# fugue-project/fugue

Hardware: NVIDIA H100
Metric: transform() rows/sec, hash-partitioned (num=256) identity map, 8-col table (higher is better)
Workload: dtype int64+f64 (byte moves; u64 hash arithmetic)

## Files before the change

fugue_b200/csrc/fb_partition.cu:

```cuda
#include <stdlib.h>

#include <mutex>

#include "fb_common.cuh"

namespace {

constexpr int kBlock = 512;
constexpr int kItems = 8;
constexpr int kTile = kBlock * kItems;
constexpr int kWarps = kBlock / 32;
constexpr int kCtasPerSm = 2;

struct FbCols {
  const void* src[FB_MAX_COLS];
  void* dst[FB_MAX_COLS];
  int32_t width[FB_MAX_COLS];
  int32_t ncols;
};

struct ChunkGeom {
  int64_t nrows;
  int64_t full_rows;
  int64_t tiles_per_chunk;
// ... 433 lines not shown

template <bool kSingleU64, int kBits, bool kAll8>
__global__ void __launch_bounds__(kBlock, kCtasPerSm)
fb_scatter_kernel(FbKeys keys, FbDiv dv, uint32_t num, ChunkGeom g, int chunk0,
                  const uint32_t* __restrict__ chunk_base, const int64_t* __restrict__ part_offsets,
                  FbCols cols) {
  extern __shared__ __align__(128) uint64_t smem64[];
  TileCtx cx;
  cx.nbp = nb_padded(num);
  cx.buf = smem64;
  cx.delta = (uint32_t*)(smem64 + 2 * kTile);
  cx.cursor = cx.delta + cx.nbp;
  cx.bin_start = cx.cursor + cx.nbp;
  cx.cnt = cx.bin_start + cx.nbp;
  cx.scanw = cx.cnt + kWarps * cx.nbp;
  cx.pid_sorted = (uint16_t*)(cx.scanw + 32);

  const int chunk = chunk0 + (int)blockIdx.x;
  int64_t chunk_row0, chunk_row1;
  chunk_range(g, chunk, chunk_row0, chunk_row1);

  for (uint32_t b = threadIdx.x; b < cx.nbp; b += kBlock)
    cx.cursor[b] = b < num ? (uint32_t)part_offsets[b] + chunk_base[(size_t)chunk * num + b] : 0u;
  for (uint32_t i = threadIdx.x; i < (uint32_t)kWarps * cx.nbp; i += kBlock) cx.cnt[i] = 0;
  __syncthreads();

  int phase = 0;
  for (int64_t tile_row0 = chunk_row0; tile_row0 < chunk_row1; tile_row0 += kTile) {
    const int64_t left = chunk_row1 - tile_row0;
    if (left >= kTile)
      scatter_tile<kSingleU64, kBits, true, kAll8>(keys, dv, num, cols, cx, tile_row0, kTile, phase);
    else
      scatter_tile<kSingleU64, kBits, false, kAll8>(keys, dv, num, cols, cx, tile_row0, (int)left, phase);
  }
}

constexpr int kSwcMaxCols = 8;
constexpr uint32_t kSwcMaxNum = 256;

__device__ __forceinline__ uint32_t smem_u32(const void* p) { return (uint32_t)__cvta_generic_to_shared(p); }

__device__ __forceinline__ void mbar_init(uint32_t bar, uint32_t count) {
  asm volatile("mbarrier.init.shared::cta.b64 [%0], %1;" ::"r"(bar), "r"(count) : "memory");
}
__device__ __forceinline__ void mbar_expect_tx(uint32_t bar, uint32_t bytes) {
  asm volatile("mbarrier.arrive.expect_tx.shared::cta.b64 _, [%0], %1;" ::"r"(bar), "r"(bytes) : "memory");
}
__device__ __forceinline__ void mbar_arrive_relaxed(uint32_t bar) {
  asm volatile("mbarrier.arrive.relaxed.cta.shared::cta.b64 _, [%0];" ::"r"(bar) : "memory");
}
__device__ __forceinline__ void mbar_wait(uint32_t bar, uint32_t parity) {
  asm volatile(
      "{\n"
      ".reg .pred p;\n"
      "FB_WAIT:\n"
      "mbarrier.try_wait.parity.shared::cta.b64 p, [%0], %1;\n"
      "@p bra FB_DONE;\n"
      "bra FB_WAIT;\n"
      "FB_DONE:\n"
      "}\n" ::"r"(bar), "r"(parity)
      : "memory");
}
__device__ __forceinline__ uint64_t l2_policy_evict_first() {
  uint64_t pol;
  asm volatile("createpolicy.fractional.L2::evict_first.b64 %0, 1.0;" : "=l"(pol));
  return pol;
}
__device__ __forceinline__ uint64_t l2_policy_evict_last() {
  uint64_t pol;
  asm volatile("createpolicy.fractional.L2::evict_last.b64 %0, 1.0;" : "=l"(pol));
  return pol;
}
__device__ __forceinline__ void tma_load_1d(uint32_t dst_smem, const void* src, uint32_t bytes, uint32_t bar,
                                            uint64_t policy) {
  asm volatile(
      "cp.async.bulk.shared::cluster.global.mbarrier::complete_tx::bytes.L2::cache_hint [%0], [%1], %2, [%3], %4;"
      ::"r"(dst_smem), "l"(src), "r"(bytes), "r"(bar), "l"(policy)
      : "memory");
}

constexpr int kWsMoverWarps = 16, kWsRankWarps = 8;
constexpr int kWsMovers = kWsMoverWarps * 32, kWsRankers = kWsRankWarps * 32;
constexpr int kWsThreads = kWsMovers + kWsRankers + 128;
constexpr int kWsG = 4;
constexpr int kWsRankItems = 16;

struct WsUnits {
  const uint64_t* src[FB_MAX_COLS];
  uint64_t* dst[FB_MAX_COLS];
  int32_t nunits;
  int32_t per_group;
  int32_t ngroups;
};

struct WsMap {
  const uint64_t* src2[FB_MAX_COLS];
  uint64_t a[FB_MAX_COLS], b[FB_MAX_COLS], c[FB_MAX_COLS];
  int32_t mode[FB_MAX_COLS];
};

__device__ __forceinline__ uint64_t ws_apply_map(int mode, bool two, uint64_t x, uint64_t y, uint64_t a, uint64_t b,
                                                 uint64_t c) {
  if (mode == 1) {
    double r = __dmul_rn(__longlong_as_double((long long)a), __longlong_as_double((long long)x));
    if (two) r = __dadd_rn(r, __dmul_rn(__longlong_as_double((long long)b), __longlong_as_double((long long)y)));
    return (uint64_t)__double_as_longlong(__dadd_rn(r, __longlong_as_double((long long)c)));
  }
  if (mode == 2) return a * x + (two ? b * y : 0ULL) + c;
  return x;
}

template <int G, int RI>
__host__ __device__ inline size_t ws_book_bytes(uint32_t num, int ncols) {
  constexpr size_t kT = (size_t)kWsRankers * RI;
  const size_t nbp = nb_padded(num);
  const size_t E = (size_t)num * (G - 1);
  size_t b = 64 * 8;
  b += (size_t)ncols * E * 8;
  b += (kT + E) * 4;
  b += 6 * nbp * 4 + 64 * 4;
  b += ((E * 2 + 15) / 16) * 16;
  b += 2 * (size_t)kMetaBytes + 128;
  return b;
}

__device__ __forceinline__ void mbar_arrive(uint32_t bar) {
  asm volatile("mbarrier.arrive.shared::cta.b64 _, [%0];" ::"r"(bar) : "memory");
}
__device__ __forceinline__ void mover_sync() { asm volatile("bar.sync 1, %0;" ::"n"(kWsMovers) : "memory"); }
__device__ __forceinline__ void ranker_sync() { asm volatile("bar.sync 2, %0;" ::"n"(kWsRankers) : "memory"); }

template <int kBits, int G, int kWsRankItems, bool kMap>
__global__ void __launch_bounds__(kWsThreads, 1)
fb_scatter_ws_kernel(WsUnits units, uint32_t num, ChunkGeom g, int nstages,
                     const uint8_t* __restrict__ meta,
                     const uint32_t* __restrict__ chunk_base, const int64_t* __restrict__ part_offsets,
                     const __grid_constant__ WsMap map) {
  constexpr uint32_t T = (uint32_t)kWsRankers * kWsRankItems;
  static_assert(T == (uint32_t)kTile, "pass 1 ranks tiles of kTile rows");
  constexpr uint32_t GM = G - 1;
  constexpr uint32_t kStageBytes = T * 8;
  constexpr int kSlotRounds = ((int)T + (int)kSwcMaxNum * (G - 1) + kWsMovers - 1) / kWsMovers;
  constexpr int kEntryRoundsM = ((int)kSwcMaxNum * (G - 1) + kWsMovers - 1) / kWsMovers;
  constexpr int kEntryRoundsR = ((int)kSwcMaxNum * (G - 1) + kWsRankers - 1) / kWsRankers;
  extern __shared__ __align__(128) uint64_t smem64[];
  const uint32_t nbp = nb_padded(num);
  const uint32_t E = num * GM;
  const int grp = (int)blockIdx.x % units.ngroups;
  const int chunk_first = (int)blockIdx.x / units.ngroups, chunk_step = (int)gridDim.x / units.ngroups;
  const int u0 = grp * units.per_group;
  const int ncols = min(units.per_group, units.nunits - u0);
  uint64_t* ring = smem64;
  uint64_t* bars = ring + (size_t)nstages * T;
  uint64_t* carry = bars + 64;
  uint32_t* slotinfo = (uint32_t*)(carry + (size_t)ncols * E);
  uint32_t* wpos = slotinfo + T + E;
  uint32_t* kcnt = wpos + nbp;
  uint32_t* binfo = kcnt + nbp;
  uint32_t* bin_n = binfo + nbp;
  uint32_t* wstart = bin_n + nbp;
  uint32_t* wdelta = wstart + nbp;
  uint32_t* scanw = wdelta + nbp;
  uint16_t* carryinfo = (uint16_t*)(scanw + 64);
  uint8_t* metabuf = (uint8_t*)(((uintptr_t)(carryinfo + E) + 127) & ~(uintptr_t)127);

  const unsigned lane = threadIdx.x & 31, warp = threadIdx.x >> 5;
  const uint32_t bar_full = smem_u32(bars), bar_empty = smem_u32(bars + 16);
  const uint32_t bar_pid_full = smem_u32(bars + 32), bar_pid_empty = smem_u32(bars + 34);
  const uint32_t bar_slots_ready = smem_u32(bars + 36), bar_slots_free = smem_u32(bars + 37);
  const uint32_t bar_flush_done = smem_u32(bars + 38);
  const uint32_t bar_carry_read = smem_u32(bars + 40);

  if (threadIdx.x == 0) {
    for (int s = 0; s < nstages; ++s) {
      mbar_init(bar_full + 8 * s, 1);
      mbar_init(bar_empty + 8 * s, kWsMoverWarps);
    }
    for (int i = 0; i < 2; ++i) {
      mbar_init(bar_pid_full + 8 * i, 1);
      mbar_init(bar_pid_empty + 8 * i, kWsRankWarps);
    }
    mbar_init(bar_slots_ready, kWsRankWarps);
    mbar_init(bar_slots_free, kWsMoverWarps);
    mbar_init(bar_flush_done, kWsMoverWarps);
    mbar_init(bar_carry_read, kWsMoverWarps);
    mbar_init(bar_carry_read + 8, kWsMoverWarps);
    asm volatile("fence.mbarrier_init.release.cluster;" ::: "memory");
  }
  __syncthreads();

  if (warp >= kWsMoverWarps + kWsRankWarps) {
    if (warp == kWsMoverWarps + kWsRankWarps && lane == 0) {
      const uint64_t pol = l2_policy_evict_first(), meta_pol = l2_policy_evict_last();
      const uint32_t ring_s = smem_u32(ring), meta_s = smem_u32(metabuf);
      uint32_t s = 0, ph = 0, seq = 0;
      int chunk = chunk_first;
      int64_t r0 = 0, r1 = 0, t0 = 0;
      bool have = chunk < g.nchunks_full;
      if (have) { chunk_range(g, chunk, r0, r1); t0 = r0; }
      auto load_pid = [&](int64_t row0, uint32_t q) {
        const uint32_t b = q & 1, pp = (q >> 1) & 1;
        mbar_wait(bar_pid_empty + 8 * b, pp ^ 1);
        mbar_expect_tx(bar_pid_full + 8 * b, kMetaBytes);
        tma_load_1d(meta_s + b * kMetaBytes, meta + (size_t)(row0 / T) * kMetaBytes, kMetaBytes,
                    bar_pid_full + 8 * b, meta_pol);
      };
      if (have) load_pid(t0, 0);
      while (have) {
        int nchunk = chunk;
        int64_t nr0 = r0, nr1 = r1, nt0 = t0 + T;
        bool nhave = true;
        if (nt0 >= r1) {
          nchunk = chunk + chunk_step;
          nhave = nchunk < g.nchunks_full;
          if (nhave) { chunk_range(g, nchunk, nr0, nr1); nt0 = nr0; }
        }
        if (nhave) load_pid(nt0, seq + 1);
        for (int u = u0; u < u0 + ncols; ++u) {
          mbar_wait(bar_empty + 8 * s, ph ^ 1);
          mbar_expect_tx(bar_full + 8 * s, kStageBytes);
          tma_load_1d(ring_s + s * kStageBytes, units.src[u] + t0, kStageBytes, bar_full + 8 * s, pol);
          if (++s == (uint32_t)nstages) { s = 0; ph ^= 1; }
          if constexpr (kMap) {
            if (map.src2[u] != nullptr) {
              mbar_wait(bar_empty + 8 * s, ph ^ 1);
              mbar_expect_tx(bar_full + 8 * s, kStageBytes);
              tma_load_1d(ring_s + s * kStageBytes, map.src2[u] + t0, kStageBytes, bar_full + 8 * s, pol);
              if (++s == (uint32_t)nstages) { s = 0; ph ^= 1; }
            }
          }
        }
        chunk = nchunk; r0 = nr0; r1 = nr1; t0 = nt0; have = nhave;
        ++seq;
      }
    }
    return;
  }

  if (warp >= kWsMoverWarps) {
    const unsigned rw = warp - kWsMoverWarps;
    const unsigned rtid = threadIdx.x - kWsMovers;
    uint32_t seq = 0, cseq = 0;
    for (int chunk = chunk_first; chunk < g.nchunks_full; chunk += chunk_step, ++cseq) {
      int64_t r0, r1;
      chunk_range(g, chunk, r0, r1);
      if (cseq > 0) mbar_wait(bar_flush_done, (cseq - 1) & 1);
      ranker_sync();
      for (uint32_t b = rtid; b < nbp; b += kWsRankers) {
        const uint32_t p0 = b < num ? (uint32_t)part_offsets[b] + chunk_base[(size_t)chunk * num + b] : 0u;
        wpos[b] = p0 & ~GM;
        kcnt[b] = (p0 & GM) | ((p0 & GM) << 8);
      }
      ranker_sync();
      for (int64_t t0 = r0; t0 < r1; t0 += T, ++seq) {
        const uint32_t pb = seq & 1, pph = (seq >> 1) & 1;
        mbar_wait(bar_pid_full + 8 * pb, pph);
        const uint8_t* __restrict__ rec = metabuf + pb * kMetaBytes;
        uint32_t pr[kWsRankItems];
#pragma unroll
        for (int r = 0; r < kWsRankItems; ++r) {
          const uint32_t row = r * kWsRankers + rtid;
          pr[r] = ((uint32_t)rec[row] << 16) | ((const uint16_t*)(rec + kMetaRank))[row];
        }
        const uint32_t b = rtid;
        uint32_t n = 0, w = 0, kold = 0, phold = 0, wp_old = 0;
        if (b < num) n = ((const uint16_t*)(rec + kMetaCnt))[b];
        __syncwarp();
        if (lane == 0) mbar_arrive_relaxed(bar_pid_empty + 8 * pb);
        if (b < num) {
          const uint32_t kc = kcnt[b];
          kold = kc & 0xFFu;
          phold = kc >> 8;
          wp_old = wpos[b];
          const uint32_t end = wp_old + kold + n;
          const uint32_t aend = end & ~GM;
          if (aend > wp_old) {
            w = aend - wp_old;
            wpos[b] = aend;
            kcnt[b] = end - aend;
          } else {
            kcnt[b] = (kold + n) | (phold << 8);
          }
          binfo[b] = kold | (phold << 4) | (w << 8);
          bin_n[b] = n;
        }
        uint32_t xw = w;
#pragma unroll
        for (int o = 1; o < 32; o <<= 1) {
          const uint32_t yw = __shfl_up_sync(0xFFFFFFFFu, xw, o);
          if (lane >= (unsigned)o) xw += yw;
        }
        if (lane == 31) scanw[8 + rw] = xw;
        ranker_sync();
        uint32_t bw = xw - w;
        {
          const uint32_t tw = lane < kWsRankWarps ? scanw[8 + lane] : 0;
#pragma unroll
          for (int wi = 0; wi < kWsRankWarps; ++wi) {
            const uint32_t vw = __shfl_sync(0xFFFFFFFFu, tw, wi);
            if ((unsigned)wi < rw) bw += vw;
          }
        }
        if (seq > 0) mbar_wait(bar_slots_free, (seq - 1) & 1);
        if (b < num) {
          wstart[b] = bw;
          wdelta[b] = wp_old - bw;
        }
        if (rtid == kWsRankers - 1) scanw[40] = bw + w;
        ranker_sync();
#pragma unroll
        for (int r = 0; r < kWsRankItems; ++r) {
          const uint32_t pb2 = pr[r] >> 16;
          const uint32_t bi = binfo[pb2];
          const uint32_t i = (bi & 0xFu) + (pr[r] & 0xFFFFu);
          const uint32_t ww = bi >> 8;
          const uint32_t row = r * kWsRankers + rtid;
          if (i < ww) slotinfo[wstart[pb2] + i] = (pb2 << 16) | row;
          else carryinfo[pb2 * GM + (i - ww)] = (uint16_t)row;
        }
#pragma unroll
        for (int q = 0; q < kEntryRoundsR; ++q) {
          const uint32_t e = q * kWsRankers + rtid;
          if (e < E) {
            const uint32_t eb = e / GM, i = e - eb * GM;
            const uint32_t bi = binfo[eb];
            const uint32_t ko = bi & 0xFu, po = (bi >> 4) & 0xFu, ww = bi >> 8;
            const uint32_t nn = bin_n[eb];
            const uint32_t desc = i < po ? 0xFFFFu : T + e;
            if (i < ko) {
              if (i < ww) slotinfo[wstart[eb] + i] = (eb << 16) | desc;
              else carryinfo[e] = (uint16_t)desc;
            }
            if (ww + i >= ko + nn) carryinfo[e] = 0xFFFFu;
          }
        }
        ranker_sync();
        if (lane == 0) mbar_arrive(bar_slots_ready);
      }
    }
    return;
  }

  uint32_t s = 0, ph = 0, seq = 0, astep = 0, wstep = 0;
  for (int chunk = chunk_first; chunk < g.nchunks_full; chunk += chunk_step) {
    int64_t r0, r1;
    chunk_range(g, chunk, r0, r1);
    for (int64_t t0 = r0; t0 < r1; t0 += T, ++seq) {
      mbar_wait(bar_slots_ready, seq & 1);
      const uint32_t W = scanw[40];
      uint32_t srcd[kSlotRounds], dst[kSlotRounds];
#pragma unroll
      for (int k = 0; k < kSlotRounds; ++k) {
        const uint32_t j = k * kWsMovers + threadIdx.x;
        srcd[k] = 0xFFFFu;
        dst[k] = 0;
        if (j < W) {
          const uint32_t info = slotinfo[j];
          srcd[k] = info & 0xFFFFu;
          dst[k] = wdelta[info >> 16] + j;
        }
      }
      uint32_t csrc[kEntryRoundsM];
#pragma unroll
      for (int q = 0; q < kEntryRoundsM; ++q) {
        const uint32_t e = q * kWsMovers + threadIdx.x;
        csrc[q] = e < E ? (uint32_t)carryinfo[e] : 0xFFFFu;
      }
      __syncwarp();
      if (lane == 0) mbar_arrive(bar_slots_free);

      uint64_t cv_prev[kEntryRoundsM];
      for (int u = 0; u < ncols; ++u) {
        mbar_wait(bar_full + 8 * s, ph);
        const uint64_t* __restrict__ st = ring + (size_t)s * T;
        uint64_t* __restrict__ out = units.dst[u0 + u];
        const uint64_t* __restrict__ cbuf = carry + (size_t)u * E;
        uint64_t v[kSlotRounds], cv[kEntryRoundsM];
        uint32_t s2 = s;
        bool two = false;
        if constexpr (kMap) {
          const int mode = map.mode[u0 + u];
          two = map.src2[u0 + u] != nullptr;
          const uint64_t* __restrict__ st2 = st;
          if (two) {
            s2 = s + 1 == (uint32_t)nstages ? 0 : s + 1;
            mbar_wait(bar_full + 8 * s2, s2 == 0 ? ph ^ 1 : ph);
            st2 = ring + (size_t)s2 * T;
          }
          const uint64_t ma = map.a[u0 + u], mb = map.b[u0 + u], mc = map.c[u0 + u];
#pragma unroll
          for (int k = 0; k < kSlotRounds; ++k)
            if (srcd[k] != 0xFFFFu)
              v[k] = srcd[k] < T ? ws_apply_map(mode, two, st[srcd[k]], st2[srcd[k]], ma, mb, mc) : cbuf[srcd[k] - T];
#pragma unroll
          for (int q = 0; q < kEntryRoundsM; ++q)
            if (csrc[q] != 0xFFFFu)
              cv[q] = csrc[q] < T ? ws_apply_map(mode, two, st[csrc[q]], st2[csrc[q]], ma, mb, mc) : cbuf[csrc[q] - T];
        } else {
#pragma unroll
          for (int k = 0; k < kSlotRounds; ++k)
            if (srcd[k] != 0xFFFFu) v[k] = srcd[k] < T ? st[srcd[k]] : cbuf[srcd[k] - T];
#pragma unroll
          for (int q = 0; q < kEntryRoundsM; ++q)
            if (csrc[q] != 0xFFFFu) cv[q] = csrc[q] < T ? st[csrc[q]] : cbuf[csrc[q] - T];
        }
#pragma unroll
        for (int k = 0; k < kSlotRounds; ++k)
          if (srcd[k] != 0xFFFFu) out[dst[k]] = v[k];
        __syncwarp();
        if (lane == 0) {
          mbar_arrive_relaxed(bar_empty + 8 * s);
          if (kMap && two) mbar_arrive_relaxed(bar_empty + 8 * s2);
          mbar_arrive_relaxed(bar_carry_read + 8 * (astep & 1));
        }
        ++astep;
        if (++s == (uint32_t)nstages) { s = 0; ph ^= 1; }
        if (kMap && two) {
          if (++s == (uint32_t)nstages) { s = 0; ph ^= 1; }
        }
        if (u > 0) {
          mbar_wait(bar_carry_read + 8 * (wstep & 1), (wstep >> 1) & 1);
          ++wstep;
          uint64_t* __restrict__ pbuf = carry + (size_t)(u - 1) * E;
#pragma unroll
          for (int q = 0; q < kEntryRoundsM; ++q) {
            const uint32_t e = q * kWsMovers + threadIdx.x;
            if (csrc[q] != 0xFFFFu) pbuf[e] = cv_prev[q];
          }
        }
#pragma unroll
        for (int q = 0; q < kEntryRoundsM; ++q) cv_prev[q] = cv[q];
      }
      {
        mbar_wait(bar_carry_read + 8 * (wstep & 1), (wstep >> 1) & 1);
        ++wstep;
        uint64_t* __restrict__ pbuf = carry + (size_t)(ncols - 1) * E;
#pragma unroll
        for (int q = 0; q < kEntryRoundsM; ++q) {
          const uint32_t e = q * kWsMovers + threadIdx.x;
          if (csrc[q] != 0xFFFFu) pbuf[e] = cv_prev[q];
        }
      }
    }
    mover_sync();
    for (int u = 0; u < ncols; ++u) {
      uint64_t* __restrict__ out = units.dst[u0 + u];
      const uint64_t* __restrict__ cbuf = carry + (size_t)u * E;
#pragma unroll
      for (int q = 0; q < kEntryRoundsM; ++q) {
        const uint32_t e = q * kWsMovers + threadIdx.x;
        if (e < E) {
          const uint32_t b = e / GM, i = e - b * GM;
          const uint32_t kc = kcnt[b];
          if (i < (kc & 0xFFu) && i >= (kc >> 8)) out[wpos[b] + i] = cbuf[e];
        }
      }
    }
    __syncwarp();
    if (lane == 0) mbar_arrive(bar_flush_done);
  }
}

__global__ void fb_bits_to_bytes_kernel(const uint8_t* __restrict__ bits, int64_t bit_offset,
                                        int64_t nrows, uint8_t* __restrict__ out) {
  int64_t i = (int64_t)blockIdx.x * blockDim.x + threadIdx.x;
  int64_t stride = (int64_t)gridDim.x * blockDim.x;
  for (; i < nrows; i += stride) {
    int64_t j = i + bit_offset;
    out[i] = (bits[j >> 3] >> (j & 7)) & 1;
  }
}

__global__ void fb_bytes_to_bits_kernel(const uint8_t* __restrict__ bytes, int64_t nrows,
                                        uint8_t* __restrict__ out, unsigned long long* null_count) {
  int64_t nbytes = (nrows + 7) >> 3;
  int64_t i = (int64_t)blockIdx.x * blockDim.x + threadIdx.x;
  int64_t stride = (int64_t)gridDim.x * blockDim.x;
  unsigned long long nulls = 0;
  for (; i < nbytes; i += stride) {
    uint8_t v = 0;
#pragma unroll
    for (int k = 0; k < 8; ++k) {
      int64_t r = i * 8 + k;
      if (r < nrows) {
        if (bytes[r]) v |= (uint8_t)(1u << k);
        else ++nulls;
      }
    }
    out[i] = v;
  }
  if (null_count != nullptr && nulls) atomicAdd(null_count, nulls);
}

inline int bits_for(uint32_t num) { return num <= 16 ? 4 : (num <= 256 ? 8 : 10); }

#define FB_DISPATCH_SB(single, bits, LAUNCH)                 \
  do {                                                       \
    if (single) {                                            \
      if (bits == 4) LAUNCH(true, 4);                        \
      else if (bits == 8) LAUNCH(true, 8);                   \
      else LAUNCH(true, 10);                                 \
    } else {                                                 \
      if (bits == 4) LAUNCH(false, 4);                       \
      else if (bits == 8) LAUNCH(false, 8);                  \
      else LAUNCH(false, 10);                                \
    }                                                        \
  } while (0)

template <typename K>
cudaError_t optin(K kernel, size_t bytes) {
  return cudaFuncSetAttribute(kernel, cudaFuncAttributeMaxDynamicSharedMemorySize, (int)bytes);
}

cudaError_t ensure_smem_optin(int dev) {
  static std::mutex mu;
  static uint64_t done = 0;
  std::lock_guard<std::mutex> lock(mu);
  if (dev >= 0 && dev < 64 && (done >> dev) & 1) return cudaSuccess;
  const size_t sc = scatter_smem_bytes(FB_MAX_PARTITIONS);
  const size_t hs = (size_t)kHistWarps * FB_MAX_PARTITIONS * sizeof(uint32_t);
  cudaError_t e = cudaSuccess;
#define FB_OPTIN(S, B)                                                   \
  do {                                                                   \
    if (e == cudaSuccess) e = optin(fb_scatter_kernel<S, B, true>, sc);  \
    if (e == cudaSuccess) e = optin(fb_scatter_kernel<S, B, false>, sc); \
    if (e == cudaSuccess) e = optin(fb_hist_kernel<S, B>, hs);           \
  } while (0)
  {
    int smem_max = 0;
    if (e == cudaSuccess) e = cudaDeviceGetAttribute(&smem_max, cudaDevAttrMaxSharedMemoryPerBlockOptin, dev);
    if (e == cudaSuccess) e = optin(fb_scatter_ws_kernel<4, kWsG, kWsRankItems, false>, (size_t)smem_max);
    if (e == cudaSuccess) e = optin(fb_scatter_ws_kernel<8, kWsG, kWsRankItems, false>, (size_t)smem_max);
    if (e == cudaSuccess) e = optin(fb_scatter_ws_kernel<4, kWsG, kWsRankItems, true>, (size_t)smem_max);
    if (e == cudaSuccess) e = optin(fb_scatter_ws_kernel<8, kWsG, kWsRankItems, true>, (size_t)smem_max);
  }
  if (e == cudaSuccess) e = optin(fb_rank_kernel<true, 4, true>, kRankStageBytes);
  if (e == cudaSuccess) e = optin(fb_rank_kernel<true, 8, true>, kRankStageBytes);
  if (e == cudaSuccess) e = optin(fb_rank_kernel<false, 4, true>, kRankStageBytes);
  if (e == cudaSuccess) e = optin(fb_rank_kernel<false, 8, true>, kRankStageBytes);
  FB_OPTIN(true, 4); FB_OPTIN(true, 8); FB_OPTIN(true, 10);
  FB_OPTIN(false, 4); FB_OPTIN(false, 8); FB_OPTIN(false, 10);
#undef FB_OPTIN
  if (e == cudaSuccess && dev >= 0 && dev < 64) done |= (1ull << dev);
  return e;
}

bool single_u64_key(int nkeys, const int32_t* widths, const uint8_t* const* valid) {
  return nkeys == 1 && widths[0] == 8 && (valid == nullptr || valid[0] == nullptr);
}

int fill_keys(FbKeys& k, int nkeys, const void* const* ptrs, const int32_t* widths,
              const uint8_t* const* valid) {
  FB_CHECK(nkeys >= 1 && nkeys <= FB_MAX_KEYS, "nkeys=%d out of range [1,%d]", nkeys, FB_MAX_KEYS);
  memset(&k, 0, sizeof(k));
  k.nkeys = nkeys;
  k.digit_shift = -1;
  for (int i = 0; i < nkeys; ++i) {
    FB_CHECK(widths[i] == 1 || widths[i] == 2 || widths[i] == 4 || widths[i] == 8,
             "key %d has unsupported width %d", i, widths[i]);
    FB_CHECK(ptrs[i] != nullptr, "key %d pointer is NULL", i);
    k.ptr[i] = ptrs[i];
    k.width[i] = widths[i];
    k.valid[i] = valid ? valid[i] : nullptr;
  }
  return 0;
}

struct PlanLayout {
  size_t hist_bytes;
  size_t pid_offset;
  size_t total_bytes;
};

PlanLayout plan_layout(const ChunkGeom& g, uint32_t num) {
  PlanLayout l;
  l.hist_bytes = (((size_t)g.nchunks * num * sizeof(uint32_t)) + 255) & ~(size_t)255;
  l.pid_offset = l.hist_bytes + 256;
  l.total_bytes = l.pid_offset + (num <= kSwcMaxNum ? (size_t)(g.full_rows / kTile) * kMetaBytes : 0) + 256;
  return l;
}

}

extern "C" {

size_t fb_partition_scratch_bytes(int dev, int64_t nrows, uint32_t num_partitions) {
  if (nrows < 0 || num_partitions == 0) return 0;
  ChunkGeom g = make_geom(dev, nrows);
  return plan_layout(g, num_partitions).total_bytes;
}

int fb_partition_ids(int dev, void* stream, int64_t nrows, int nkeys, const void* const* key_ptrs,
                     const int32_t* key_widths, const uint8_t* const* key_valid,
                     uint32_t num_partitions, uint32_t* out_pids) {
  FB_CHECK(nrows >= 0, "nrows < 0");
  FB_CHECK(num_partitions >= 1, "num_partitions must be >= 1");
  if (nrows == 0) return 0;
  FbDeviceGuard guard(dev);
  FB_CHECK(guard.ok, "cannot select device %d", dev);
  FbKeys k;
  if (int rc = fill_keys(k, nkeys, key_ptrs, key_widths, key_valid)) return rc;
  FbDiv dv = fb_make_div(num_partitions);
  int64_t blocks = (nrows + 255) / 256;
  int64_t maxb = (int64_t)fb_sm_count(dev) * 16;
  if (blocks > maxb) blocks = maxb;
  cudaStream_t st = (cudaStream_t)stream;
  if (single_u64_key(nkeys, key_widths, key_valid))
    fb_pid_kernel<true><<<(unsigned)blocks, 256, 0, st>>>(k, dv, nrows, out_pids);
  else
    fb_pid_kernel<false><<<(unsigned)blocks, 256, 0, st>>>(k, dv, nrows, out_pids);
  FB_CUDA(cudaGetLastError());
  return 0;
}

int fb_row_hash64(int dev, void* stream, int64_t nrows, int nkeys, const void* const* key_ptrs,
                  const int32_t* key_widths, const uint8_t* const* key_valid, uint64_t* out_hash) {
  FB_CHECK(nrows >= 0, "nrows < 0");
// ... 105 lines not shown
                      const int32_t* col_widths, void* const* out_col_ptrs, int sm_reserve = 0,
                      const fb_map_unit* maps = nullptr, void* tail_tmp = nullptr, int cols_per_launch_req = 0) {
  FB_CHECK(nrows >= 0 && nrows < ((int64_t)1 << 32), "nrows out of range");
  FB_CHECK(num_partitions >= 1 && num_partitions <= FB_MAX_PARTITIONS,
           "num_partitions=%u out of range [1,%d]", num_partitions, FB_MAX_PARTITIONS);
  FB_CHECK(ncols >= 0, "ncols < 0");
  if (nrows == 0 || ncols == 0) return 0;
  FbDeviceGuard guard(dev);
  FB_CHECK(guard.ok, "cannot select device %d", dev);
  ChunkGeom g = make_geom(dev, nrows);
  PlanLayout l = plan_layout(g, num_partitions);
  FB_CHECK(scratch != nullptr && scratch_bytes >= l.total_bytes, "scratch too small");
  FbDiv dv = fb_make_div(num_partitions);
  cudaStream_t st = (cudaStream_t)stream;
  const size_t smem = scatter_smem_bytes(num_partitions);
  FB_CUDA(ensure_smem_optin(dev));
  const int bits = bits_for(num_partitions);

  for (int c = 0; c < ncols; ++c) {
    const int w = col_widths[c];
    FB_CHECK(w == 1 || w == 2 || w == 4 || w == 8, "column %d has unsupported width %d", c, w);
    FB_CHECK(col_ptrs[c] != nullptr && out_col_ptrs[c] != nullptr, "column %d pointer is NULL", c);
  }

  const void* const* gen_src = col_ptrs;
  auto launch_generic = [&](const int* idx, int n, int chunk0, int nch) -> int {
    for (int c0 = 0; c0 < n && nch > 0; c0 += FB_MAX_COLS) {
      FbCols cols;
      memset(&cols, 0, sizeof(cols));
      cols.ncols = n - c0 < FB_MAX_COLS ? n - c0 : FB_MAX_COLS;
      bool all8 = true;
      for (int c = 0; c < cols.ncols; ++c) {
        cols.src[c] = gen_src[idx[c0 + c]];
        cols.dst[c] = out_col_ptrs[idx[c0 + c]];
        cols.width[c] = col_widths[idx[c0 + c]];
        all8 = all8 && cols.width[c] == 8;
      }
#define FB_LAUNCH_SCATTER(S, B)                                                                        \
  do {                                                                                                 \
    if (all8)                                                                                          \
      fb_scatter_kernel<S, B, true><<<nch, kBlock, smem, st>>>(k, dv, num_partitions, g, chunk0,       \
                                                               (const uint32_t*)scratch, part_offsets, cols); \
    else                                                                                               \
      fb_scatter_kernel<S, B, false><<<nch, kBlock, smem, st>>>(k, dv, num_partitions, g, chunk0,      \
                                                                (const uint32_t*)scratch, part_offsets, cols); \
  } while (0)
      FB_DISPATCH_SB(single, bits, FB_LAUNCH_SCATTER);
#undef FB_LAUNCH_SCATTER
      FB_CUDA(cudaGetLastError());
    }
    return 0;
  };

  const bool fast_ok = num_partitions <= kSwcMaxNum && g.nchunks_full > 0;
  if (maps != nullptr) {
    FB_CHECK(num_partitions <= kSwcMaxNum, "fused map needs num_partitions <= %u", kSwcMaxNum);
    FB_CHECK(tail_tmp != nullptr || g.full_rows == nrows, "fused map: tail_tmp is NULL");
    for (int c = 0; c < ncols; ++c) {
      FB_CHECK(col_widths[c] == 8 && (uintptr_t)col_ptrs[c] % 16 == 0, "fused map: column %d is not an aligned 8-byte column", c);
      FB_CHECK(maps[c].mode >= 0 && maps[c].mode <= 2, "fused map: column %d has mode %d", c, maps[c].mode);
      FB_CHECK(maps[c].src2 == nullptr || (maps[c].mode != 0 && (uintptr_t)maps[c].src2 % 16 == 0),
               "fused map: bad second operand of column %d", c);
    }
  }
  int* fast_idx = (int*)alloca(sizeof(int) * (size_t)ncols);
  int* gen_idx = (int*)alloca(sizeof(int) * (size_t)ncols);
  int nfast = 0, ngen = 0;
  for (int c = 0; c < ncols; ++c) {
    if (fast_ok && col_widths[c] == 8 && (uintptr_t)col_ptrs[c] % 16 == 0) fast_idx[nfast++] = c;
    else gen_idx[ngen++] = c;
  }
  if (int rc = launch_generic(gen_idx, ngen, 0, g.nchunks)) return rc;

  if (nfast > 0) {
    int smem_max = 0;
    FB_CUDA(cudaDeviceGetAttribute(&smem_max, cudaDevAttrMaxSharedMemoryPerBlockOptin, dev));
    int avail = fb_sm_count(dev) - sm_reserve;
    if (avail < 1) avail = 1;
    const uint8_t* pid_plane = (const uint8_t*)scratch + l.pid_offset;
    int ngroups = (nfast + 1) / 2;
    int per_group = (nfast + ngroups - 1) / ngroups;
    if (cols_per_launch_req >= 1 && cols_per_launch_req <= kSwcMaxCols) per_group = cols_per_launch_req;
    ngroups = (nfast + per_group - 1) / per_group;
    const size_t book = ws_book_bytes<kWsG, kWsRankItems>(num_partitions, per_group);
    const size_t stage_bytes = (size_t)kWsRankers * kWsRankItems * 8;
    int nstages = (int)(((size_t)smem_max - book) / stage_bytes);
    if (nstages > 16) nstages = 16;
    FB_CHECK(nstages >= 2, "not enough shared memory for the TMA ring (%d stages)", nstages);
    const size_t tsmem = (size_t)nstages * stage_bytes + book;
    const int groups_per_launch = ngroups <= avail ? (ngroups < FB_MAX_COLS / per_group ? ngroups : FB_MAX_COLS / per_group) : 1;
    for (int g0 = 0; g0 < ngroups; g0 += groups_per_launch) {
      const int lg = ngroups - g0 < groups_per_launch ? ngroups - g0 : groups_per_launch;
      const int c0 = g0 * per_group;
      const int nu = nfast - c0 < lg * per_group ? nfast - c0 : lg * per_group;
      WsUnits wu;
      WsMap wm;
      memset(&wu, 0, sizeof(wu));
      memset(&wm, 0, sizeof(wm));
      wu.nunits = nu;
      wu.per_group = per_group;
      wu.ngroups = lg;
      for (int c = 0; c < nu; ++c) {
        wu.src[c] = (const uint64_t*)col_ptrs[fast_idx[c0 + c]];
        wu.dst[c] = (uint64_t*)out_col_ptrs[fast_idx[c0 + c]];
        if (maps != nullptr) {
          const fb_map_unit& m = maps[fast_idx[c0 + c]];
          wm.src2[c] = (const uint64_t*)m.src2;
          wm.a[c] = m.a; wm.b[c] = m.b; wm.c[c] = m.c;
          wm.mode[c] = m.mode;
        }
      }
      const int64_t ctas = avail < (int64_t)lg * g.nchunks_full ? avail : (int64_t)lg * g.nchunks_full;
      const int grid = (int)(ctas / lg) * lg;
      if (maps != nullptr) {
        if (bits == 4)
          fb_scatter_ws_kernel<4, kWsG, kWsRankItems, true><<<grid, kWsThreads, tsmem, st>>>(
              wu, num_partitions, g, nstages, pid_plane, (const uint32_t*)scratch, part_offsets, wm);
        else
          fb_scatter_ws_kernel<8, kWsG, kWsRankItems, true><<<grid, kWsThreads, tsmem, st>>>(
              wu, num_partitions, g, nstages, pid_plane, (const uint32_t*)scratch, part_offsets, wm);
      } else if (bits == 4) {
        fb_scatter_ws_kernel<4, kWsG, kWsRankItems, false><<<grid, kWsThreads, tsmem, st>>>(
            wu, num_partitions, g, nstages, pid_plane, (const uint32_t*)scratch, part_offsets, wm);
      } else {
        fb_scatter_ws_kernel<8, kWsG, kWsRankItems, false><<<grid, kWsThreads, tsmem, st>>>(
            wu, num_partitions, g, nstages, pid_plane, (const uint32_t*)scratch, part_offsets, wm);
      }
      FB_CUDA(cudaGetLastError());
    }
    if (maps == nullptr)
      if (int rc = launch_generic(fast_idx, nfast, g.nchunks_full, g.nchunks - g.nchunks_full)) return rc;
  }
  if (maps != nullptr && g.full_rows < nrows) {
    FB_CHECK(ncols <= kSwcMaxCols * 8, "fused map: too many columns (%d)", ncols);
    uint8_t* base = (uint8_t*)tail_tmp;
    const size_t hdr = (((size_t)ncols * (sizeof(void*) + sizeof(fb_map_unit))) + 255) & ~(size_t)255;
    FB_CUDA(cudaMemcpyAsync(base, col_ptrs, sizeof(void*) * (size_t)ncols, cudaMemcpyHostToDevice, st));
    FB_CUDA(cudaMemcpyAsync(base + sizeof(void*) * (size_t)ncols, maps, sizeof(fb_map_unit) * (size_t)ncols,
                            cudaMemcpyHostToDevice, st));
    uint64_t* vals = (uint64_t*)(base + hdr);
    fb_map_tail_kernel<<<32, 256, 0, st>>>(ncols, (const void* const*)base,
                                           (const fb_map_unit*)(base + sizeof(void*) * (size_t)ncols), g.full_rows,
                                           nrows, vals);
    FB_CUDA(cudaGetLastError());
    const void** shifted = (const void**)alloca(sizeof(void*) * (size_t)ncols);
    int* all_idx = (int*)alloca(sizeof(int) * (size_t)ncols);
    for (int c = 0; c < ncols; ++c) {
      shifted[c] = (const uint8_t*)(vals + (size_t)c * kTile) - (size_t)g.full_rows * 8;
      all_idx[c] = c;
    }
    gen_src = shifted;
    if (int rc = launch_generic(all_idx, ncols, g.nchunks_full, g.nchunks - g.nchunks_full)) return rc;
  }
  return 0;
}

int fb_partition_apply(int dev, void* stream, int64_t nrows, int nkeys, const void* const* key_ptrs,
                       const int32_t* key_widths, const uint8_t* const* key_valid,
                       uint32_t num_partitions, const void* scratch, size_t scratch_bytes,
                       const int64_t* part_offsets, int ncols, const void* const* col_ptrs,
                       const int32_t* col_widths, void* const* out_col_ptrs) {
  if (nrows == 0 || ncols == 0) return 0;
  FbKeys k;
  if (int rc = fill_keys(k, nkeys, key_ptrs, key_widths, key_valid)) return rc;
  return apply_impl(dev, stream, nrows, k, single_u64_key(nkeys, key_widths, key_valid), num_partitions,
                    scratch, scratch_bytes, part_offsets, ncols, col_ptrs, col_widths, out_col_ptrs);
}

int fb_partition_apply_ex(int dev, void* stream, int64_t nrows, int nkeys, const void* const* key_ptrs,
                          const int32_t* key_widths, const uint8_t* const* key_valid,
                          uint32_t num_partitions, const void* scratch, size_t scratch_bytes,
                          const int64_t* part_offsets, int ncols, const void* const* col_ptrs,
                          const int32_t* col_widths, void* const* out_col_ptrs, int sm_reserve,
                          int cols_per_launch) {
  if (nrows == 0 || ncols == 0) return 0;
  FB_CHECK(sm_reserve >= 0, "sm_reserve < 0");
  FbKeys k;
  if (int rc = fill_keys(k, nkeys, key_ptrs, key_widths, key_valid)) return rc;
  return apply_impl(dev, stream, nrows, k, single_u64_key(nkeys, key_widths, key_valid), num_partitions,
                    scratch, scratch_bytes, part_offsets, ncols, col_ptrs, col_widths, out_col_ptrs, sm_reserve,
                    nullptr, nullptr, cols_per_launch);
}

size_t fb_partition_map_tail_bytes(int ncols) {
  if (ncols < 0) return 0;
  return ((((size_t)ncols * (sizeof(void*) + sizeof(fb_map_unit))) + 255) & ~(size_t)255) + (size_t)ncols * kTile * 8;
}

int fb_partition_apply_map(int dev, void* stream, int64_t nrows, int nkeys, const void* const* key_ptrs,
                           const int32_t* key_widths, const uint8_t* const* key_valid,
                           uint32_t num_partitions, const void* scratch, size_t scratch_bytes,
                           const int64_t* part_offsets, int ncols, const void* const* col_ptrs,
                           void* const* out_col_ptrs, const fb_map_unit* maps, void* tail_tmp, int sm_reserve) {
  if (nrows == 0 || ncols == 0) return 0;
  FB_CHECK(maps != nullptr, "maps is NULL");
  FB_CHECK(ncols <= FB_MAX_COLS, "ncols=%d > %d", ncols, FB_MAX_COLS);
  FbKeys k;
  if (int rc = fill_keys(k, nkeys, key_ptrs, key_widths, key_valid)) return rc;
  int32_t widths[FB_MAX_COLS];
  for (int c = 0; c < ncols; ++c) widths[c] = 8;
  return apply_impl(dev, stream, nrows, k, single_u64_key(nkeys, key_widths, key_valid), num_partitions,
                    scratch, scratch_bytes, part_offsets, ncols, col_ptrs, widths, out_col_ptrs, sm_reserve, maps,
                    tail_tmp);
}

int fb_radix_pass(int dev, void* stream, int64_t nrows, const void* sort_key_u64, int shift, int ncols,
                  const void* const* col_ptrs, const int32_t* col_widths, void* const* out_col_ptrs,
                  void* scratch, size_t scratch_bytes, int64_t* d_offsets ) {
  FB_CHECK(shift >= 0 && shift <= 56, "shift out of range");
  if (nrows == 0) return 0;
// ... 60 lines not shown
```

Before: 16.61 billion.

## Rebalance warp-specialized scatter registers, widen write granularity, simplify carry bookkeeping

Warp roles now use setmaxnreg to shift registers from the TMA producer and ranker warps to the mover warps. When two columns are handled per group and shared memory allows, a wider group size (G=16) is used, so each partition flushes larger contiguous runs. The ranker reads per-row metadata from shared memory rather than holding it in registers, and processes its carry entries per bin, which drops the bin_n array. Movers now write carry values in place after a mover barrier instead of using double-buffered carry-read mbarriers. The cost is a larger carry buffer and fewer ring stages for G=16, plus an extra block-wide barrier per column.

```diff
diff --git a/fugue_b200/csrc/fb_partition.cu b/fugue_b200/csrc/fb_partition.cu
--- a/fugue_b200/csrc/fb_partition.cu
+++ b/fugue_b200/csrc/fb_partition.cu
@@ -539,8 +539,14 @@
 constexpr int kWsMoverWarps = 16, kWsRankWarps = 8;
 constexpr int kWsMovers = kWsMoverWarps * 32, kWsRankers = kWsRankWarps * 32;
 constexpr int kWsThreads = kWsMovers + kWsRankers + 128;
-constexpr int kWsG = 4;
+constexpr int kWsG = 16;
+constexpr int kWsGWide = 4;
+constexpr int kWsMinStages = 3;
 constexpr int kWsRankItems = 16;
+constexpr uint32_t kWsProducerRegs = 24, kWsRankerRegs = 64, kWsMoverRegs = 88;
+static_assert(128 * kWsProducerRegs + kWsRankers * kWsRankerRegs + kWsMovers * kWsMoverRegs <= kWsThreads * 72,
+              "setmaxnreg: the roles take more registers than the launch gives the CTA");
+constexpr int kMoveBatch = 8;
 
 struct WsUnits {
   const uint64_t* src[FB_MAX_COLS];
@@ -575,7 +581,7 @@
   size_t b = 64 * 8;
   b += (size_t)ncols * E * 8;
   b += (kT + E) * 4;
-  b += 6 * nbp * 4 + 64 * 4;
+  b += 5 * nbp * 4 + 64 * 4;
   b += ((E * 2 + 15) / 16) * 16;
   b += 2 * (size_t)kMetaBytes + 128;
   return b;
@@ -586,6 +592,10 @@
 }
 __device__ __forceinline__ void mover_sync() { asm volatile("bar.sync 1, %0;" ::"n"(kWsMovers) : "memory"); }
 __device__ __forceinline__ void ranker_sync() { asm volatile("bar.sync 2, %0;" ::"n"(kWsRankers) : "memory"); }
+template <uint32_t N>
+__device__ __forceinline__ void setmaxnreg_dec() { asm volatile("setmaxnreg.dec.sync.aligned.u32 %0;" ::"n"(N)); }
+template <uint32_t N>
+__device__ __forceinline__ void setmaxnreg_inc() { asm volatile("setmaxnreg.inc.sync.aligned.u32 %0;" ::"n"(N)); }
 
 template <int kBits, int G, int kWsRankItems, bool kMap>
 __global__ void __launch_bounds__(kWsThreads, 1)
@@ -595,11 +605,11 @@
                      const __grid_constant__ WsMap map) {
   constexpr uint32_t T = (uint32_t)kWsRankers * kWsRankItems;
   static_assert(T == (uint32_t)kTile, "pass 1 ranks tiles of kTile rows");
+  static_assert(G >= 2 && G <= 16 && (G & (G - 1)) == 0, "G must be a power of two <= 16");
   constexpr uint32_t GM = G - 1;
   constexpr uint32_t kStageBytes = T * 8;
   constexpr int kSlotRounds = ((int)T + (int)kSwcMaxNum * (G - 1) + kWsMovers - 1) / kWsMovers;
   constexpr int kEntryRoundsM = ((int)kSwcMaxNum * (G - 1) + kWsMovers - 1) / kWsMovers;
-  constexpr int kEntryRoundsR = ((int)kSwcMaxNum * (G - 1) + kWsRankers - 1) / kWsRankers;
   extern __shared__ __align__(128) uint64_t smem64[];
   const uint32_t nbp = nb_padded(num);
   const uint32_t E = num * GM;
@@ -614,8 +624,7 @@
   uint32_t* wpos = slotinfo + T + E;
   uint32_t* kcnt = wpos + nbp;
   uint32_t* binfo = kcnt + nbp;
-  uint32_t* bin_n = binfo + nbp;
-  uint32_t* wstart = bin_n + nbp;
+  uint32_t* wstart = binfo + nbp;
   uint32_t* wdelta = wstart + nbp;
   uint32_t* scanw = wdelta + nbp;
   uint16_t* carryinfo = (uint16_t*)(scanw + 64);
@@ -626,7 +635,6 @@
   const uint32_t bar_pid_full = smem_u32(bars + 32), bar_pid_empty = smem_u32(bars + 34);
   const uint32_t bar_slots_ready = smem_u32(bars + 36), bar_slots_free = smem_u32(bars + 37);
   const uint32_t bar_flush_done = smem_u32(bars + 38);
-  const uint32_t bar_carry_read = smem_u32(bars + 40);
 
   if (threadIdx.x == 0) {
     for (int s = 0; s < nstages; ++s) {
@@ -640,13 +648,12 @@
     mbar_init(bar_slots_ready, kWsRankWarps);
     mbar_init(bar_slots_free, kWsMoverWarps);
     mbar_init(bar_flush_done, kWsMoverWarps);
-    mbar_init(bar_carry_read, kWsMoverWarps);
-    mbar_init(bar_carry_read + 8, kWsMoverWarps);
     asm volatile("fence.mbarrier_init.release.cluster;" ::: "memory");
   }
   __syncthreads();
 
   if (warp >= kWsMoverWarps + kWsRankWarps) {
+    setmaxnreg_dec<kWsProducerRegs>();
     if (warp == kWsMoverWarps + kWsRankWarps && lane == 0) {
       const uint64_t pol = l2_policy_evict_first(), meta_pol = l2_policy_evict_last();
       const uint32_t ring_s = smem_u32(ring), meta_s = smem_u32(metabuf);
@@ -695,6 +702,7 @@
   }
 
   if (warp >= kWsMoverWarps) {
+    setmaxnreg_dec<kWsRankerRegs>();
     const unsigned rw = warp - kWsMoverWarps;
     const unsigned rtid = threadIdx.x - kWsMovers;
     uint32_t seq = 0, cseq = 0;
@@ -713,17 +721,9 @@
         const uint32_t pb = seq & 1, pph = (seq >> 1) & 1;
         mbar_wait(bar_pid_full + 8 * pb, pph);
         const uint8_t* __restrict__ rec = metabuf + pb * kMetaBytes;
-        uint32_t pr[kWsRankItems];
-#pragma unroll
-        for (int r = 0; r < kWsRankItems; ++r) {
-          const uint32_t row = r * kWsRankers + rtid;
-          pr[r] = ((uint32_t)rec[row] << 16) | ((const uint16_t*)(rec + kMetaRank))[row];
-        }
         const uint32_t b = rtid;
         uint32_t n = 0, w = 0, kold = 0, phold = 0, wp_old = 0;
         if (b < num) n = ((const uint16_t*)(rec + kMetaCnt))[b];
-        __syncwarp();
-        if (lane == 0) mbar_arrive_relaxed(bar_pid_empty + 8 * pb);
         if (b < num) {
           const uint32_t kc = kcnt[b];
           kold = kc & 0xFFu;
@@ -738,8 +738,7 @@
           } else {
             kcnt[b] = (kold + n) | (phold << 8);
           }
-          binfo[b] = kold | (phold << 4) | (w << 8);
-          bin_n[b] = n;
+          binfo[b] = kold | (w << 8);
         }
         uint32_t xw = w;
 #pragma unroll
@@ -767,28 +766,26 @@
         ranker_sync();
 #pragma unroll
         for (int r = 0; r < kWsRankItems; ++r) {
-          const uint32_t pb2 = pr[r] >> 16;
+          const uint32_t row = r * kWsRankers + rtid;
+          const uint32_t pb2 = rec[row];
           const uint32_t bi = binfo[pb2];
-          const uint32_t i = (bi & 0xFu) + (pr[r] & 0xFFFFu);
+          const uint32_t i = (bi & 0xFFu) + ((const uint16_t*)(rec + kMetaRank))[row];
           const uint32_t ww = bi >> 8;
-          const uint32_t row = r * kWsRankers + rtid;
           if (i < ww) slotinfo[wstart[pb2] + i] = (pb2 << 16) | row;
           else carryinfo[pb2 * GM + (i - ww)] = (uint16_t)row;
         }
-#pragma unroll
-        for (int q = 0; q < kEntryRoundsR; ++q) {
-          const uint32_t e = q * kWsRankers + rtid;
-          if (e < E) {
-            const uint32_t eb = e / GM, i = e - eb * GM;
-            const uint32_t bi = binfo[eb];
-            const uint32_t ko = bi & 0xFu, po = (bi >> 4) & 0xFu, ww = bi >> 8;
-            const uint32_t nn = bin_n[eb];
-            const uint32_t desc = i < po ? 0xFFFFu : T + e;
-            if (i < ko) {
-              if (i < ww) slotinfo[wstart[eb] + i] = (eb << 16) | desc;
+        __syncwarp();
+        if (lane == 0) mbar_arrive_relaxed(bar_pid_empty + 8 * pb);
+        if (b < num) {
+#pragma unroll
+          for (uint32_t i = 0; i < GM; ++i) {
+            const uint32_t e = b * GM + i;
+            const uint32_t desc = i < phold ? 0xFFFFu : T + e;
+            if (i < kold) {
+              if (i < w) slotinfo[bw + i] = (b << 16) | desc;
               else carryinfo[e] = (uint16_t)desc;
             }
-            if (ww + i >= ko + nn) carryinfo[e] = 0xFFFFu;
+            if (w + i >= kold + n) carryinfo[e] = 0xFFFFu;
           }
         }
         ranker_sync();
@@ -798,7 +795,8 @@
     return;
   }
 
-  uint32_t s = 0, ph = 0, seq = 0, astep = 0, wstep = 0;
+  setmaxnreg_inc<kWsMoverRegs>();
+  uint32_t s = 0, ph = 0, seq = 0;
   for (int chunk = chunk_first; chunk < g.nchunks_full; chunk += chunk_step) {
     int64_t r0, r1;
     chunk_range(g, chunk, r0, r1);
@@ -821,83 +819,62 @@
 #pragma unroll
       for (int q = 0; q < kEntryRoundsM; ++q) {
         const uint32_t e = q * kWsMovers + threadIdx.x;
-        csrc[q] = e < E ? (uint32_t)carryinfo[e] : 0xFFFFu;
+        const uint32_t d = e < E ? (uint32_t)carryinfo[e] : 0xFFFFu;
+        csrc[q] = d < T ? d : 0xFFFFu;
       }
       __syncwarp();
       if (lane == 0) mbar_arrive(bar_slots_free);
 
-      uint64_t cv_prev[kEntryRoundsM];
       for (int u = 0; u < ncols; ++u) {
         mbar_wait(bar_full + 8 * s, ph);
         const uint64_t* __restrict__ st = ring + (size_t)s * T;
         uint64_t* __restrict__ out = units.dst[u0 + u];
-        const uint64_t* __restrict__ cbuf = carry + (size_t)u * E;
-        uint64_t v[kSlotRounds], cv[kEntryRoundsM];
+        uint64_t* __restrict__ cbuf = carry + (size_t)u * E;
         uint32_t s2 = s;
         bool two = false;
+        const uint64_t* __restrict__ st2 = st;
+        int mode = 0;
+        uint64_t ma = 0, mb = 0, mc = 0;
         if constexpr (kMap) {
-          const int mode = map.mode[u0 + u];
+          mode = map.mode[u0 + u];
           two = map.src2[u0 + u] != nullptr;
-          const uint64_t* __restrict__ st2 = st;
           if (two) {
             s2 = s + 1 == (uint32_t)nstages ? 0 : s + 1;
             mbar_wait(bar_full + 8 * s2, s2 == 0 ? ph ^ 1 : ph);
             st2 = ring + (size_t)s2 * T;
           }
-          const uint64_t ma = map.a[u0 + u], mb = map.b[u0 + u], mc = map.c[u0 + u];
-#pragma unroll
-          for (int k = 0; k < kSlotRounds; ++k)
-            if (srcd[k] != 0xFFFFu)
-              v[k] = srcd[k] < T ? ws_apply_map(mode, two, st[srcd[k]], st2[srcd[k]], ma, mb, mc) : cbuf[srcd[k] - T];
-#pragma unroll
-          for (int q = 0; q < kEntryRoundsM; ++q)
-            if (csrc[q] != 0xFFFFu)
-              cv[q] = csrc[q] < T ? ws_apply_map(mode, two, st[csrc[q]], st2[csrc[q]], ma, mb, mc) : cbuf[csrc[q] - T];
-        } else {
-#pragma unroll
-          for (int k = 0; k < kSlotRounds; ++k)
-            if (srcd[k] != 0xFFFFu) v[k] = srcd[k] < T ? st[srcd[k]] : cbuf[srcd[k] - T];
-#pragma unroll
-          for (int q = 0; q < kEntryRoundsM; ++q)
-            if (csrc[q] != 0xFFFFu) cv[q] = csrc[q] < T ? st[csrc[q]] : cbuf[csrc[q] - T];
-        }
-#pragma unroll
-        for (int k = 0; k < kSlotRounds; ++k)
-          if (srcd[k] != 0xFFFFu) out[dst[k]] = v[k];
+          ma = map.a[u0 + u]; mb = map.b[u0 + u]; mc = map.c[u0 + u];
+        }
+        auto staged = [&](uint32_t r) -> uint64_t {
+          if constexpr (kMap) return ws_apply_map(mode, two, st[r], st2[r], ma, mb, mc);
+          else return st[r];
+        };
+#pragma unroll
+        for (int k0 = 0; k0 < kSlotRounds; k0 += kMoveBatch) {
+          uint64_t v[kMoveBatch];
+#pragma unroll
+          for (int k = 0; k < kMoveBatch; ++k)
+            if (k0 + k < kSlotRounds && srcd[k0 + k] != 0xFFFFu)
+              v[k] = srcd[k0 + k] < T ? staged(srcd[k0 + k]) : cbuf[srcd[k0 + k] - T];
+#pragma unroll
+          for (int k = 0; k < kMoveBatch; ++k)
+            if (k0 + k < kSlotRounds && srcd[k0 + k] != 0xFFFFu) out[dst[k0 + k]] = v[k];
+        }
+        mover_sync();
+#pragma unroll
+        for (int q = 0; q < kEntryRoundsM; ++q)
+          if (csrc[q] != 0xFFFFu) cbuf[q * kWsMovers + threadIdx.x] = staged(csrc[q]);
         __syncwarp();
         if (lane == 0) {
           mbar_arrive_relaxed(bar_empty + 8 * s);
           if (kMap && two) mbar_arrive_relaxed(bar_empty + 8 * s2);
-          mbar_arrive_relaxed(bar_carry_read + 8 * (astep & 1));
-        }
-        ++astep;
+        }
         if (++s == (uint32_t)nstages) { s = 0; ph ^= 1; }
         if (kMap && two) {
           if (++s == (uint32_t)nstages) { s = 0; ph ^= 1; }
         }
-        if (u > 0) {
-          mbar_wait(bar_carry_read + 8 * (wstep & 1), (wstep >> 1) & 1);
-          ++wstep;
-          uint64_t* __restrict__ pbuf = carry + (size_t)(u - 1) * E;
-#pragma unroll
-          for (int q = 0; q < kEntryRoundsM; ++q) {
-            const uint32_t e = q * kWsMovers + threadIdx.x;
-            if (csrc[q] != 0xFFFFu) pbuf[e] = cv_prev[q];
-          }
-        }
-#pragma unroll
-        for (int q = 0; q < kEntryRoundsM; ++q) cv_prev[q] = cv[q];
-      }
-      {
-        mbar_wait(bar_carry_read + 8 * (wstep & 1), (wstep >> 1) & 1);
-        ++wstep;
-        uint64_t* __restrict__ pbuf = carry + (size_t)(ncols - 1) * E;
-#pragma unroll
-        for (int q = 0; q < kEntryRoundsM; ++q) {
-          const uint32_t e = q * kWsMovers + threadIdx.x;
-          if (csrc[q] != 0xFFFFu) pbuf[e] = cv_prev[q];
-        }
-      }
+      }
+      if (ncols == 1) mover_sync();
     }
     mover_sync();
     for (int u = 0; u < ncols; ++u) {
@@ -986,10 +963,16 @@
   {
     int smem_max = 0;
     if (e == cudaSuccess) e = cudaDeviceGetAttribute(&smem_max, cudaDevAttrMaxSharedMemoryPerBlockOptin, dev);
-    if (e == cudaSuccess) e = optin(fb_scatter_ws_kernel<4, kWsG, kWsRankItems, false>, (size_t)smem_max);
-    if (e == cudaSuccess) e = optin(fb_scatter_ws_kernel<8, kWsG, kWsRankItems, false>, (size_t)smem_max);
-    if (e == cudaSuccess) e = optin(fb_scatter_ws_kernel<4, kWsG, kWsRankItems, true>, (size_t)smem_max);
-    if (e == cudaSuccess) e = optin(fb_scatter_ws_kernel<8, kWsG, kWsRankItems, true>, (size_t)smem_max);
+#define FB_OPTIN_WS(G)                                                                                        \
+  do {                                                                                                        \
+    if (e == cudaSuccess) e = optin(fb_scatter_ws_kernel<4, G, kWsRankItems, false>, (size_t)smem_max);       \
+    if (e == cudaSuccess) e = optin(fb_scatter_ws_kernel<8, G, kWsRankItems, false>, (size_t)smem_max);       \
+    if (e == cudaSuccess) e = optin(fb_scatter_ws_kernel<4, G, kWsRankItems, true>, (size_t)smem_max);        \
+    if (e == cudaSuccess) e = optin(fb_scatter_ws_kernel<8, G, kWsRankItems, true>, (size_t)smem_max);        \
+  } while (0)
+    FB_OPTIN_WS(kWsG);
+    FB_OPTIN_WS(kWsGWide);
+#undef FB_OPTIN_WS
   }
   if (e == cudaSuccess) e = optin(fb_rank_kernel<true, 4, true>, kRankStageBytes);
   if (e == cudaSuccess) e = optin(fb_rank_kernel<true, 8, true>, kRankStageBytes);
@@ -1261,9 +1244,13 @@
     int per_group = (nfast + ngroups - 1) / ngroups;
     if (cols_per_launch_req >= 1 && cols_per_launch_req <= kSwcMaxCols) per_group = cols_per_launch_req;
     ngroups = (nfast + per_group - 1) / per_group;
-    const size_t book = ws_book_bytes<kWsG, kWsRankItems>(num_partitions, per_group);
     const size_t stage_bytes = (size_t)kWsRankers * kWsRankItems * 8;
-    int nstages = (int)(((size_t)smem_max - book) / stage_bytes);
+    auto stages_for = [&](size_t book) { return book < (size_t)smem_max ? (int)(((size_t)smem_max - book) / stage_bytes) : 0; };
+    const bool lines = per_group == 2 &&
+                       stages_for(ws_book_bytes<kWsG, kWsRankItems>(num_partitions, per_group)) >= kWsMinStages;
+    const size_t book = lines ? ws_book_bytes<kWsG, kWsRankItems>(num_partitions, per_group)
+                              : ws_book_bytes<kWsGWide, kWsRankItems>(num_partitions, per_group);
+    int nstages = stages_for(book);
     if (nstages > 16) nstages = 16;
     FB_CHECK(nstages >= 2, "not enough shared memory for the TMA ring (%d stages)", nstages);
     const size_t tsmem = (size_t)nstages * stage_bytes + book;
@@ -1291,20 +1278,24 @@
       }
       const int64_t ctas = avail < (int64_t)lg * g.nchunks_full ? avail : (int64_t)lg * g.nchunks_full;
       const int grid = (int)(ctas / lg) * lg;
-      if (maps != nullptr) {
-        if (bits == 4)
-          fb_scatter_ws_kernel<4, kWsG, kWsRankItems, true><<<grid, kWsThreads, tsmem, st>>>(
-              wu, num_partitions, g, nstages, pid_plane, (const uint32_t*)scratch, part_offsets, wm);
-        else
-          fb_scatter_ws_kernel<8, kWsG, kWsRankItems, true><<<grid, kWsThreads, tsmem, st>>>(
-              wu, num_partitions, g, nstages, pid_plane, (const uint32_t*)scratch, part_offsets, wm);
-      } else if (bits == 4) {
-        fb_scatter_ws_kernel<4, kWsG, kWsRankItems, false><<<grid, kWsThreads, tsmem, st>>>(
-            wu, num_partitions, g, nstages, pid_plane, (const uint32_t*)scratch, part_offsets, wm);
-      } else {
-        fb_scatter_ws_kernel<8, kWsG, kWsRankItems, false><<<grid, kWsThreads, tsmem, st>>>(
-            wu, num_partitions, g, nstages, pid_plane, (const uint32_t*)scratch, part_offsets, wm);
-      }
+#define FB_LAUNCH_WS(B, G, M)                                                                               \
+  fb_scatter_ws_kernel<B, G, kWsRankItems, M><<<grid, kWsThreads, tsmem, st>>>(                              \
+      wu, num_partitions, g, nstages, pid_plane, (const uint32_t*)scratch, part_offsets, wm)
+#define FB_LAUNCH_WS_G(G)                                                                                   \
+  do {                                                                                                      \
+    if (maps != nullptr) {                                                                                  \
+      if (bits == 4) FB_LAUNCH_WS(4, G, true);                                                              \
+      else FB_LAUNCH_WS(8, G, true);                                                                        \
+    } else if (bits == 4) {                                                                                 \
+      FB_LAUNCH_WS(4, G, false);                                                                            \
+    } else {                                                                                                \
+      FB_LAUNCH_WS(8, G, false);                                                                            \
+    }                                                                                                       \
+  } while (0)
+      if (lines) FB_LAUNCH_WS_G(kWsG);
+      else FB_LAUNCH_WS_G(kWsGWide);
+#undef FB_LAUNCH_WS_G
+#undef FB_LAUNCH_WS
       FB_CUDA(cudaGetLastError());
     }
     if (maps == nullptr)
```

New measurement: 17.36 billion, median of 6. 1.05x the previous value.
